# angelowxx/Super_resolution-Image-Reconstructer-Multi_Generator_GAN

Hardware: NVIDIA B200
Metric: srgan_train_lr_patches_per_sec (higher is better)
Workload: dtype bf16

## Files before the change

super_resolution-image-reconstructer-multi_generator_gan_b200/_lib.py:

```python
from __future__ import annotations

import ctypes
import os
import subprocess
from ctypes import POINTER, c_char_p, c_double, c_float, c_int, c_int64, c_longlong, c_size_t, c_void_p

HERE = os.path.dirname(os.path.abspath(__file__))
ROOT = os.path.dirname(HERE)
CSRC = os.path.join(HERE, "csrc")
SO_PATH = os.environ.get("SRG_LIB_SO") or os.path.join(HERE, "libsrgan_b200.so")
SOURCES = ["conv_gemm.cu", "conv_ops.cu", "vgg_ops.cu", "resample.cu", "trunk_fused.cu", "wgrad_gemm.cu", "elementwise.cu", "peer_sync.cu", "generator.cu", "discriminator.cu", "api.cu"]
NVCC_FLAGS = ["-gencode", "arch=compute_100a,code=sm_100a", "-O3", "-lineinfo", "-std=c++17", "-shared",
              "-Xcompiler", "-fPIC"]

_lib = None


def _sources():
    return [os.path.join(CSRC, s) for s in SOURCES if os.path.exists(os.path.join(CSRC, s))]


def needs_build() -> bool:
    if os.environ.get("SRG_LIB_SO"):
        return False
    if not os.path.exists(SO_PATH):
        return True
    so_m = os.path.getmtime(SO_PATH)
    deps = _sources() + [os.path.join(CSRC, f) for f in os.listdir(CSRC) if f.endswith(".cuh")]
    deps.append(os.path.join(ROOT, "include", "srgan_b200.h"))
    return any(os.path.getmtime(d) > so_m for d in deps if os.path.exists(d))


def build(force: bool = False, verbose: bool = False) -> str:
    if not force and not needs_build():
        return SO_PATH
    nvcc = os.environ.get("NVCC", "/usr/local/cuda/bin/nvcc")
    cmd = [nvcc] + NVCC_FLAGS + ["-o", SO_PATH] + _sources() + ["-ldl"]
    if verbose:
        print(" ".join(cmd))
    r = subprocess.run(cmd, capture_output=True, text=True)
    if r.returncode != 0:
        raise RuntimeError("nvcc failed:\n" + r.stdout + r.stderr)
    return SO_PATH

# ... 146 lines not shown
```

super_resolution-image-reconstructer-multi_generator_gan_b200/csrc/conv_gemm.cu:

```cuda
#include "conv_gemm.cuh"
#include "elementwise.cuh"
#include "launch.cuh"
#include "ptx.cuh"

#include <stdarg.h>
#include <stdlib.h>
#include <stdio.h>
#include <string.h>

namespace srg {

static thread_local char g_err[512] = "";
const char* last_error() { return g_err; }
void set_error(const char* fmt, ...) {
  va_list ap;
  va_start(ap, fmt);
  vsnprintf(g_err, sizeof(g_err), fmt, ap);
  va_end(ap);
}

static long long g_launch_total = 0;
void count_launch(int n) { __atomic_fetch_add(&g_launch_total, (long long)n, __ATOMIC_RELAXED); }
long long total_launches() { return __atomic_load_n(&g_launch_total, __ATOMIC_RELAXED); }

// ... 1140 lines not shown
                                         227 * 1024);
    if (e != cudaSuccess) { set_error("cudaFuncSetAttribute: %s", cudaGetErrorString(e)); return int(e); }
    attr_set = true;
  }
  cudaError_t e = launch_pdl(conv_gemm_kernel<BLOCK_N, NT>, grid, dim3(kThreads), smem_bytes, stream, p);
  if (e == cudaSuccess) e = cudaGetLastError();
  if (e != cudaSuccess) { set_error("conv_gemm launch: %s", cudaGetErrorString(e)); return int(e); }
  count_launch();
  return 0;
}

static bool conv3_il_enabled() {
  static int on = -1;
  if (on < 0) {
    const char* ev = getenv("SRG_CONV_IL");
    on = (ev != nullptr && ev[0] == '0') ? 0 : 1;
  }
  return on != 0;
}
static bool conv3_il_wide_enabled() {
  static int on = -1;
  if (on < 0) {
    const char* ev = getenv("SRG_CONV_IL_WIDE");
    on = (ev != nullptr && ev[0] == '0') ? 0 : 1;
  }
  return on != 0;
}
static int g_variant_override = 0;
int set_conv_variant(int variant) {
  const int old = g_variant_override;
  g_variant_override = (variant >= 0 && variant <= 3) ? variant : 0;
  return old;
}
static int effective_variant(const ConvGemmArgs& a) { return a.variant != 0 ? a.variant : g_variant_override; }
static bool use_conv3_il(const ConvGemmArgs& a) {
  const int variant = effective_variant(a);
  if (variant == 1 || (variant == 0 && !conv3_il_enabled())) return false;
  return a.TH == 16 && a.TW == 8 && a.block_n == 64 && a.n_strips == 3 && a.n_taps == 3 && a.strip_dh == -1 &&
         a.strip_rows == 18 && a.tap_row[0] == 0 && a.tap_row[1] == 1 && a.tap_row[2] == 2 && a.n_views == 1 &&
         a.views[0].channels == 64 && a.in_H == a.H && a.in_W == a.W && a.H >= 2 &&
         (a.out_mode == OUT_NHWC || a.out_mode == OUT_PIXEL_SHUFFLE) &&
         a.cout_total % 64 == 0 && a.cout_total <= 256;
}

static int encode_parity_map(CUtensorMap* map, const void* base, int C, int W, int H, int N, int64_t stride_w,
                             int64_t stride_h, int64_t stride_n, int par, uint32_t box_rows, uint32_t box_w = 8) {
  const __nv_bfloat16* ptr = reinterpret_cast<const __nv_bfloat16*>(base) + size_t(par) * stride_h;
  uint64_t dims[4] = {uint64_t(C), uint64_t(W), uint64_t((H - par + 1) / 2), uint64_t(N)};
  uint64_t strides[3] = {uint64_t(stride_w) * 2, uint64_t(stride_h) * 4, uint64_t(stride_n) * 2};
  uint32_t box[4] = {64, box_w, box_rows, 1};
  return encode_map_bf16(map, ptr, 4, dims, strides, box);
}

static int launch_conv3_il(const ConvGemmArgs* as, int n, cudaStream_t stream) {
  const ConvGemmArgs& a = as[0];
  if (n < 1 || n > kIlMaxGroups) { set_error("conv3_il: 1..%d groups", kIlMaxGroups); return -17; }
  for (int g = 1; g < n; ++g) {
    const ConvGemmArgs& o = as[g];
    if (o.N != a.N || o.H != a.H || o.W != a.W || o.in_H != a.in_H || o.in_W != a.in_W || o.cout_total != 64 || a.cout_total != 64 ||
        o.out_mode != OUT_NHWC || a.out_mode != OUT_NHWC || o.act != a.act || o.slope != a.slope || o.exclusive != a.exclusive ||
        (o.residual != nullptr) != (a.residual != nullptr) || (o.mask_src != nullptr) != (a.mask_src != nullptr) ||
        (o.stats != nullptr) != (a.stats != nullptr) || (o.stats_y != nullptr) != (a.stats_y != nullptr) ||
        o.views[0].stride_w != a.views[0].stride_w || o.views[0].stride_h != a.views[0].stride_h ||
        o.views[0].stride_n != a.views[0].stride_n || o.strip_dw[0] != a.strip_dw[0] || o.strip_dw[1] != a.strip_dw[1] ||
        o.strip_dw[2] != a.strip_dw[2] || effective_variant(o) != effective_variant(a) || a.prof != nullptr) {
      set_error("conv3_il: the problems of a grouped launch must share geometry, epilogue and layout (OUT_NHWC, 64 channels)");
// ... 349 lines not shown
```

super_resolution-image-reconstructer-multi_generator_gan_b200/csrc/conv_gemm.cuh:

```cuda
#pragma once
#include <cuda.h>
#include <cuda_bf16.h>
#include <cuda_runtime.h>
#include <stdint.h>

namespace srg {

constexpr int kMaxStrips = 9;
constexpr int kMaxTaps = 9;
constexpr int kMaxInMaps = 4;

enum ConvAct : int { ACT_NONE = 0, ACT_RELU = 1, ACT_LRELU = 2 };
enum ConvOutMode : int {
  OUT_NHWC = 0,
  OUT_PIXEL_SHUFFLE = 1,
  OUT_FOLD9_NCHW = 2,
  OUT_NHWC_F32 = 3,
};

struct InView {
  const void* ptr;
  int64_t stride_w;
  int64_t stride_h;
  int64_t stride_n;
// ... 50 lines not shown
};
int wgrad_partials_floats(const WgradArgs& a, int* splits_out);
int launch_wgrad_gemm(const WgradArgs& a, cudaStream_t stream);
int wgrad3x3_partials_floats(const WgradArgs& a, int* splits_out);
int launch_wgrad3x3(const WgradArgs& a, cudaStream_t stream);
struct WgradBatchArgs {
  int N, H, W, n_layers;
  const void* x_base;
  int64_t x_layer_stride_bytes;
  const void* dy_base;
  int64_t dy_layer_stride_bytes;
  float* partials;
  const int* inv;
  float* grads;
  const long long* out_off;
};
void wgrad3_batched_plan(const WgradBatchArgs& a, int* tiles_per_layer, int* grid, int* per_cta, int* max_slots);
size_t wgrad3_batched_partials_floats(const WgradBatchArgs& a);
int launch_wgrad3x3_batched(const WgradBatchArgs& a, cudaStream_t stream);
int launch_wgrad_reduce(const float* partials, const int* idx, float* out, int n_out, int splits, size_t split_stride,
                        int accumulate_into, cudaStream_t stream);

struct C9Window { int jlo, jhi, slot_lo, fresh; };
__host__ __device__ inline C9Window c9_window(int ri) {
  C9Window w;
  w.jlo = ri > 8 ? ri - 8 : 0;
  w.jhi = ri < 7 ? ri : 7;
  w.slot_lo = 8 - ri + w.jlo;
  w.fresh = ri <= 7 ? 1 : 0;
  return w;
}

int set_conv_variant(int variant);

int sm_budget();
void set_sm_share(int k);

void count_launch(int n = 1);
long long total_launches();

int launch_wgrad_reduce_inv(const float* partials, const int* inv, float* out, int n_part, int splits, size_t split_stride,
                            cudaStream_t stream);

const char* last_error();
void set_error(const char* fmt, ...);

}
```

super_resolution-image-reconstructer-multi_generator_gan_b200/csrc/generator.cu:

```cuda
#include "generator.cuh"

#include <stdio.h>
#include <stdlib.h>
#include <string.h>

#include "conv_gemm.cuh"
#include "elementwise.cuh"
#include "peer_sync.cuh"
#include "trunk_fused.cuh"

namespace srg {

namespace {

constexpr float kBnEps = 1e-5f;
constexpr float kBnMomentum = 0.1f;
constexpr float kSlope = 0.2f;

struct Carver {
  size_t off = 0;
  size_t take(size_t bytes) {
    const size_t o = off;
    off += (bytes + 1023) & ~size_t(1023);
    return o;
  }
};

struct Layout {
  size_t packed, bias, bncoef, bwdcoef, partials, sums, ticket, wg_partials, ps_scratch, loss_scratch;
  size_t dyall = 0, slot = 0;
  size_t wgb_partials = 0, wgb_floats = 0;
  size_t trunk_sync = 0, trunk_tab = 0;
  size_t U1, out1, trunk;
  std::vector<size_t> y1, z1, y2, out;
  std::vector<size_t> up;
  size_t g[4];
  std::vector<size_t> dup;
  size_t Ud;
// ... 40 lines not shown
    }
  } else {
    const size_t y1 = c.take(t64(P)), z1 = c.take(t64(P)), y2 = c.take(t64(P)), oa = c.take(t64(P)), ob = c.take(t64(P));
    for (int b = 0; b < e.n_res; ++b) { L.y1[b] = y1; L.z1[b] = z1; L.y2[b] = y2; L.out[b] = (b & 1) ? ob : oa; }
  }
  L.trunk = c.take(t64(P));
  L.up.resize(e.n_up);
  for (int j = 0; j < e.n_up; ++j) L.up[j] = c.take(t64(P << (2 * (j + 1))));
  L.wg_partials = L.ps_scratch = L.loss_scratch = L.Ud = 0;
  for (int i = 0; i < 4; ++i) L.g[i] = 0;
  L.dup.assign(e.n_up, 0);
  if (training) {
    L.wg_partials = c.take(size_t(wgrad_max_floats(e.n_up)) * 4);
    L.ps_scratch = c.take(size_t(e.N) * (size_t(e.H) << e.n_up) * 128 * 4);
    L.loss_scratch = c.take(size_t(loss_scratch_doubles()) * 8);
    for (int i = 0; i < 3; ++i) L.g[i] = c.take(t64(P));
    L.slot = (t64(P) + 1023) & ~size_t(1023);
    L.dyall = c.take(L.slot * size_t(2 * e.n_res + 1));
    L.g[3] = L.dyall + L.slot * size_t(2 * e.n_res);
    L.kd_last = L.kd_c1 = 0;
    if (e.keep_grads) {
      L.kd_y2.resize(e.n_res); L.kd_p1.resize(e.n_res); L.kd_y1.resize(e.n_res); L.kd_in.resize(e.n_res);
      for (int b = 0; b < e.n_res; ++b) {
        L.kd_y2[b] = L.dyall + L.slot * size_t(2 * b + 1); L.kd_y1[b] = L.dyall + L.slot * size_t(2 * b);
        L.kd_p1[b] = c.take(t64(P)); L.kd_in[b] = c.take(t64(P));
      }
      L.kd_last = c.take(t64(P));
      L.kd_c1 = c.take(t64(P));
    }
    L.wgb_floats = wgrad_batched_floats(e);
    L.wgb_partials = c.take(L.wgb_floats * 4);
    for (int j = 0; j < e.n_up; ++j) L.dup[j] = c.take(t64(P << (2 * (j + 1))));
    const int64_t Hs = int64_t(e.H) << e.n_up, Ws = int64_t(e.W) << e.n_up;
    L.Ud = c.take(size_t(e.N) * (Hs + 1) * Ws * 128);
  }
  L.total = c.off;
  return L;
}

int64_t add_param(GeneratorEngine& e, const std::string& name, std::initializer_list<int> shape) {
  ParamInfo p;
  p.name = name;
  p.ndim = int(shape.size());
  p.numel = 1;
  int i = 0;
  for (int s : shape) { p.shape[i++] = s; p.numel *= s; }
  for (; i < 4; ++i) p.shape[i] = 1;
  p.offset = e.param_elems;
  e.param_elems += (p.numel + 3) & ~int64_t(3);
  e.params.push_back(p);
  return p.offset;
}
int64_t poff(const GeneratorEngine& e, const std::string& name) {
  for (const auto& p : e.params)
    if (p.name == name) return p.offset;
  return -1;
}
int64_t boff(const GeneratorEngine& e, const std::string& name) {
  for (const auto& b : e.buffers)
    if (b.name == name) return b.offset;
  return -1;
}

struct PackOffsets {
  int64_t conv1_f;
  std::vector<int64_t> rb_f[2], rb_d[2];
  int64_t conv2_f, conv2_d;
// ... 579 lines not shown
  for (size_t i = 0; i + 1 < g->prof_used; i += 2) {
    cudaError_t e = cudaEventSynchronize(g->prof_events[i + 1]);
    if (e != cudaSuccess) { set_error("profile_read: %s", cudaGetErrorString(e)); return int(e); }
    float ms = 0.f;
    e = cudaEventElapsedTime(&ms, g->prof_events[i], g->prof_events[i + 1]);
    if (e != cudaSuccess) { set_error("profile_read: %s", cudaGetErrorString(e)); return int(e); }
    total += double(ms);
  }
  if (ms_sum) *ms_sum = total;
  if (count) *count = (long long)(g->prof_used / 2);
  g->prof_used = 0;
  return 0;
}

GeneratorEngine::~GeneratorEngine() {
  for (cudaEvent_t ev : prof_events) cudaEventDestroy(ev);
  cudaFree(d_pack_idx); cudaFree(d_bias_idx); cudaFree(d_wg_idx_c3x3); cudaFree(d_wg_idx_up);
  cudaFree(d_wg_idx_conv1); cudaFree(d_wg_idx_conv3); cudaFree(d_wgb_off);
}

GeneratorEngine* generator_create(int N, int H, int W, int n_res, int n_up) {
  if (N < 1 || H < 1 || W < 1 || n_res < 0 || n_up < 0 || n_up > 4) { set_error("generator_create: bad geometry"); return nullptr; }
  EngineImpl* e = new EngineImpl();
  e->N = N; e->H = H; e->W = W; e->n_res = n_res; e->n_up = n_up;
  {
    const char* ev = getenv("SRG_FUSE_BWD_STATS");
    e->fuse_bwd_stats = ev != nullptr && ev[0] == '1';
    ev = getenv("SRG_REDUCE_FINAL");
    e->reduce_final = ev != nullptr && ev[0] == '1';
    ev = getenv("SRG_FIN_FUSED");
    e->fin_fused = ev != nullptr && ev[0] == '1';
    ev = getenv("SRG_WGRAD_BATCHED");
    e->wgrad_batched = !(ev != nullptr && ev[0] == '0');
  }
  add_param(*e, "conv1.weight", {64, 3, 9, 9});
  add_param(*e, "conv1.bias", {64});
  char nm[96];
  for (int b = 0; b < n_res; ++b) {
    const char* sub[2][2] = {{"conv1", "bn1"}, {"conv2", "bn2"}};
    for (int k = 0; k < 2; ++k) {
      snprintf(nm, sizeof(nm), "residual_blocks.%d.%s.weight", b, sub[k][0]); add_param(*e, nm, {64, 64, 3, 3});
      snprintf(nm, sizeof(nm), "residual_blocks.%d.%s.bias", b, sub[k][0]); add_param(*e, nm, {64});
      snprintf(nm, sizeof(nm), "residual_blocks.%d.%s.weight", b, sub[k][1]); add_param(*e, nm, {64});
      snprintf(nm, sizeof(nm), "residual_blocks.%d.%s.bias", b, sub[k][1]); add_param(*e, nm, {64});
      for (const char* stat : {"running_mean", "running_var"}) {
        BufferInfo bi;
        snprintf(nm, sizeof(nm), "residual_blocks.%d.%s.%s", b, sub[k][1], stat);
        bi.name = nm; bi.offset = e->buffer_elems; bi.numel = 64;
        e->buffer_elems += 64;
        e->buffers.push_back(bi);
      }
    }
  }
  add_param(*e, "conv2.weight", {64, 64, 3, 3});
  add_param(*e, "conv2.bias", {64});
  for (int j = 0; j < n_up; ++j) {
    snprintf(nm, sizeof(nm), "upsample.%d.weight", 3 * j); add_param(*e, nm, {256, 64, 3, 3});
    snprintf(nm, sizeof(nm), "upsample.%d.bias", 3 * j); add_param(*e, nm, {256});
  }
  add_param(*e, "conv3.weight", {3, 64, 9, 9});
  add_param(*e, "conv3.bias", {3});

  std::vector<int> idx;
  idx.reserve(size_t(e->param_elems) * 2 + 65536);
  PackOffsets& po = e->po;
  po.conv1_f = int64_t(idx.size()); pack_conv1_fwd(idx, poff(*e, "conv1.weight"));
// ... 405 lines not shown
    return launch_wgrad_reduce_inv(wgp, idx, e->grads + pi->offset, int(per_split), splits, per_split, st);
  };
  auto bias_grad = [&](const void* dy, int64_t pixels, const std::string& bname) -> int {
    ReduceFinalize f; memset(&f, 0, sizeof(f));
    f.mode = RF_SUM; f.count = double(pixels); f.out0 = e->grads + poff(*e, bname);
    RC(launch_chan_reduce(dy, nullptr, pixels, partials, st));
    e->launches += 2;
    return launch_partials_finalize(partials, reduce_blocks(pixels), f, st);
  };
  int bwd_stats_rows = 0;
  auto dgrad3x3 = [&](const void* dy_base, int gh, int gw, bool dy_ps, int64_t w_off, const void* residual, const void* mask,
                      void* out, const void* stats_y) -> int {
    ConvGemmArgs a; memset(&a, 0, sizeof(a));
    a.N = N; a.H = gh; a.W = gw; set_taps_3x3(a);
    if (dy_ps) {
      a.n_views = 4;
      for (int q = 0; q < 4; ++q) a.views[q] = ps_view(dy_base, gh, gw, q);
    } else {
      a.n_views = 1; a.views[0] = plain_view(dy_base, gh, gw);
    }
    a.in_H = gh; a.in_W = gw;
    a.weights = packed + w_off; a.cout_total = 64; a.block_n = 64;
    a.bias = nullptr; a.act = ACT_NONE; a.residual = residual; a.mask_src = mask; a.out = out; a.out_mode = OUT_NHWC;
    if (stats_y != nullptr && e->fuse_bwd_stats) { a.stats = partials; a.stats_y = stats_y; bwd_stats_rows = conv_gemm_grid(a); }
    e->launches += 1;
    if (dy_ps) return launch_conv_gemm(a, st);
    ProfScope ps(e, st);
    return launch_conv_gemm(a, st);
  };

  const void* conv3_in = S > 0 ? ws + L.up[S - 1] : ws + L.trunk;
  void* d_trunk = ws + L.g[3];
  if (pre) {
  RC(launch_unfold9(dsr, N, Hs, Ws, 1.f, ws + L.Ud, st));
  RC(launch_nchw_chan_sum(dsr, N, 3, int64_t(Hs) * Ws, reinterpret_cast<double*>(ws + L.loss_scratch),
                          e->grads + poff(*e, "conv3.bias"), 1.f, st));
  e->launches += 3;
  {
    InView uv = plain_view(ws + L.Ud, Hs + 1, Ws);
    RC(wgrad(uv, Hs + 1, Ws, true, Hs, Ws, conv3_in, 1, false, e->d_wg_idx_conv3, "conv3.weight"));
  }
  {
    ConvGemmArgs a; memset(&a, 0, sizeof(a));
    a.N = N; a.H = Hs; a.W = Ws; set_taps_pairs(a);
    a.n_views = 1; a.views[0] = plain_view(ws + L.Ud, Hs + 1, Ws); a.in_H = Hs + 1; a.in_W = Ws;
    a.weights = packed + po.conv3_d; a.cout_total = 64; a.block_n = 64;
    a.act = ACT_NONE; a.out_mode = OUT_NHWC;
    a.mask_src = S > 0 ? conv3_in : nullptr;
    a.out = S > 0 ? ws + L.dup[S - 1] : d_trunk;
    RC(launch_conv_gemm(a, st));
    e->launches += 1;
  }
  for (int j = S - 1; j >= 0; --j) {
    const int Hj = H << j, Wj = W << j;
    const void* in_j = j > 0 ? ws + L.up[j - 1] : ws + L.trunk;
    snprintf(nm, sizeof(nm), "upsample.%d.bias", 3 * j);
    RC(launch_ps_bias_grad(ws + L.dup[j], N, Hj * 2, Wj * 2, reinterpret_cast<float*>(ws + L.ps_scratch),
                           e->grads + poff(*e, nm), st));
    e->launches += 2;
    snprintf(nm, sizeof(nm), "upsample.%d.weight", 3 * j);
    RC(wgrad(plain_view(in_j, Hj, Wj), Hj, Wj, false, Hj, Wj, ws + L.dup[j], 4, true, e->d_wg_idx_up, nm));
    RC(dgrad3x3(ws + L.dup[j], Hj, Wj, true, po.up_d[j], nullptr, j > 0 ? in_j : nullptr, j > 0 ? ws + L.dup[j - 1] : d_trunk, nullptr));
  }
  }
  const void* x_last = e->n_res > 0 ? ws + L.out[e->n_res - 1] : ws + L.out1;
  if (pre) RC(bias_grad(d_trunk, P, "conv2.bias"));
  bool batched = e->wgrad_batched && e->n_res > 0;
  for (int b = 0; b < e->n_res && batched; ++b) {
    const size_t x1 = b > 0 ? L.out[b - 1] : L.out1;
    if (x1 != L.out1 + size_t(2 * b) * 2 * L.slot || L.z1[b] != L.out1 + size_t(2 * b + 1) * 2 * L.slot) batched = false;
  }
  if (batched && L.out[e->n_res - 1] != L.out1 + size_t(2 * e->n_res) * 2 * L.slot) batched = false;
  if (batched) {
    WgradBatchArgs probe; memset(&probe, 0, sizeof(probe));
    probe.N = N; probe.H = H; probe.W = W; probe.n_layers = 2 * e->n_res + 1;
    if (wgrad3_batched_partials_floats(probe) > L.wgb_floats) batched = false;
  }
  if (!batched && pre) RC(wgrad(plain_view(x_last, H, W), H, W, false, H, W, d_trunk, 1, false, e->d_wg_idx_c3x3, "conv2.weight"));
  const bool keep = e->keep_grads;
  void* dout = keep ? ws + L.kd_last : ws + L.g[0];
  void* dother = ws + L.g[1];
  void* dmid = ws + L.g[2];
  const bool fused = batched && use_trunk_fused(*e);
  const bool layers_here = !fused && phases == kPhaseAll;
// ... 91 lines not shown
```

super_resolution-image-reconstructer-multi_generator_gan_b200/csrc/generator.cuh:

```cuda
#pragma once
#include <cuda_runtime.h>
#include <stdint.h>

#include <string>
#include <vector>

namespace srg {

struct ParamInfo {
  std::string name;
  int64_t offset;
  int64_t numel;
  int ndim;
  int shape[4];
};
struct BufferInfo {
  std::string name;
  int64_t offset;
  int64_t numel;
};
struct TensorInfo {
  std::string name;
  int64_t byte_offset;
  int dims[4];
// ... 2 lines not shown

typedef int (*AllreduceF64Fn)(void* ctx, double* buf, int n, cudaStream_t stream);

struct GeneratorEngine {
  int N, H, W, n_res, n_up;
  std::vector<ParamInfo> params;
  std::vector<BufferInfo> buffers;
  std::vector<TensorInfo> tensors;
  int64_t param_elems = 0, buffer_elems = 0;
  int64_t packed_elems = 0, bias_elems = 0;
  size_t workspace_bytes_train = 0, workspace_bytes_eval = 0;
  int* d_pack_idx = nullptr;
  int* d_bias_idx = nullptr;
  int* d_wg_idx_c3x3 = nullptr;
  int* d_wg_idx_up = nullptr;
  int* d_wg_idx_conv1 = nullptr;
  int* d_wg_idx_conv3 = nullptr;
  long long* d_wgb_off = nullptr;
  float* master = nullptr;
  float* grads = nullptr;
  float* bn_buffers = nullptr;
  uint8_t* ws = nullptr;
  size_t ws_bytes = 0;
  bool ws_training = false;
  AllreduceF64Fn allreduce = nullptr;
  void* allreduce_ctx = nullptr;
  struct PeerSync* peer = nullptr;
  int world = 1;
  long long launches = 0;
  bool fuse_bwd_stats = false;
  bool fin_fused = false;
  bool reduce_final = false;
  bool wgrad_batched = true;
  bool keep_grads = false;
  bool prof_on = false;
  std::vector<cudaEvent_t> prof_events;
  size_t prof_used = 0;
  int prof_layers = 1;

  virtual ~GeneratorEngine();
};

GeneratorEngine* generator_create(int N, int H, int W, int n_res, int n_up);
int generator_bind(GeneratorEngine* g, float* master, float* grads, float* bn_buffers, void* ws, size_t ws_bytes,
                   int training);
int generator_pack(GeneratorEngine* g, cudaStream_t st);
int generator_forward(GeneratorEngine* g, const float* lr_nchw, float* sr_nchw, int training, int update_running,
                      cudaStream_t st);
int generator_backward(GeneratorEngine* g, const float* dsr_nchw, cudaStream_t st);
enum GeneratorPhase : int { kPhasePre = 1, kPhaseTrunk = 2, kPhasePost = 4, kPhaseAll = 7 };
int generator_forward_phases(GeneratorEngine* g, const float* lr_nchw, float* sr_nchw, int training, int update_running,
                             int phases, cudaStream_t st);
int generator_backward_phases(GeneratorEngine* g, const float* dsr_nchw, int phases, cudaStream_t st);
int generators_trunk(GeneratorEngine* const* gs, int n, int bwd, int update_running, cudaStream_t st);
int generator_set_keep_grads(GeneratorEngine* g, int keep);
int generator_trunk_error(GeneratorEngine* g);
int generator_prof_layers(const GeneratorEngine* g);
int generator_profile_enable(GeneratorEngine* g, int on);
int generator_profile_read(GeneratorEngine* g, double* ms_sum, long long* count);

}
```

Before: 1702.

## Fuse conv3 backward unfold into dedicated dgrad and wgrad tcgen05 kernels

New measurement: 1750, median of 6. +2.8%, better.

```diff
diff --git a/super_resolution-image-reconstructer-multi_generator_gan_b200/_lib.py b/super_resolution-image-reconstructer-multi_generator_gan_b200/_lib.py
--- a/super_resolution-image-reconstructer-multi_generator_gan_b200/_lib.py
+++ b/super_resolution-image-reconstructer-multi_generator_gan_b200/_lib.py
@@ -9,7 +9,7 @@
 ROOT = os.path.dirname(HERE)
 CSRC = os.path.join(HERE, "csrc")
 SO_PATH = os.environ.get("SRG_LIB_SO") or os.path.join(HERE, "libsrgan_b200.so")
-SOURCES = ["conv_gemm.cu", "conv_ops.cu", "vgg_ops.cu", "resample.cu", "trunk_fused.cu", "wgrad_gemm.cu", "elementwise.cu", "peer_sync.cu", "generator.cu", "discriminator.cu", "api.cu"]
+SOURCES = ["conv_gemm.cu", "conv_ops.cu", "vgg_ops.cu", "resample.cu", "trunk_fused.cu", "wgrad_gemm.cu", "conv9_bwd.cu", "elementwise.cu", "peer_sync.cu", "generator.cu", "discriminator.cu", "api.cu"]
 NVCC_FLAGS = ["-gencode", "arch=compute_100a,code=sm_100a", "-O3", "-lineinfo", "-std=c++17", "-shared",
               "-Xcompiler", "-fPIC"]
 
diff --git a/super_resolution-image-reconstructer-multi_generator_gan_b200/csrc/conv9_bwd.cu b/super_resolution-image-reconstructer-multi_generator_gan_b200/csrc/conv9_bwd.cu
--- /dev/null
+++ b/super_resolution-image-reconstructer-multi_generator_gan_b200/csrc/conv9_bwd.cu
@@ -0,0 +1,551 @@
+#include "conv9_bwd.cuh"
+#include "elementwise.cuh"
+#include "launch.cuh"
+#include "ptx.cuh"
+
+#include <string.h>
+
+namespace srg {
+
+int encode_map_bf16(CUtensorMap* map, const void* ptr, int rank, const uint64_t* dims, const uint64_t* strides_bytes,
+                    const uint32_t* box);
+
+namespace {
+
+constexpr int kTH = 16, kTW = 8;
+constexpr int kStripRows = 24;
+constexpr uint32_t kStripBytes = kStripRows * kTW * 128;
+constexpr uint32_t kTileBytes = kTH * kTW * 128;
+constexpr int kWinRows = kStripRows + 1;
+constexpr int kWinCols = 16;
+constexpr int kWinPitch = 24;
+constexpr int kWinPlane = kWinRows * kWinPitch;
+constexpr int kWinLoads = 3 * kWinRows * kWinCols;
+constexpr uint32_t kWinBytes = 3 * kWinPlane * 4;
+constexpr int kBuilders = 192;
+constexpr int kPf = (kWinLoads + kBuilders - 1) / kBuilders;
+constexpr int kTaps = 5;
+constexpr uint32_t kWBytes = kTaps * 64 * 128;
+
+struct TileXY { int n, h0, w0; };
+__device__ __forceinline__ TileXY tile_xy(int tile, int tiles_w, int tiles_per_img) {
+  TileXY t;
+  t.n = tile / tiles_per_img;
+  const int rem = tile - t.n * tiles_per_img;
+  t.h0 = (rem / tiles_w) * kTH;
+  t.w0 = (rem % tiles_w) * kTW;
+  return t;
+}
+
+__device__ __forceinline__ void win_prefetch(float (&pf)[kPf], const float* __restrict__ dsr, int H, int W, int btid, TileXY t,
+                                             bool valid) {
+#pragma unroll
+  for (int k = 0; k < kPf; ++k) {
+    const int i = btid + k * kBuilders;
+    const int c = i / (kWinRows * kWinCols);
+    const int rem = i - c * (kWinRows * kWinCols);
+    const int r = rem / kWinCols, col = rem - r * kWinCols;
+    const int hh = t.h0 - 4 + r, ww = t.w0 - 4 + col;
+    pf[k] = (valid && i < kWinLoads && hh >= 0 && hh < H && ww >= 0 && ww < W)
+                ? __ldg(dsr + ((size_t(t.n) * 3 + c) * H + hh) * size_t(W) + ww) : 0.f;
+  }
+}
+__device__ __forceinline__ void win_store(const float (&pf)[kPf], float* win, int btid) {
+#pragma unroll
+  for (int k = 0; k < kPf; ++k) {
+    const int i = btid + k * kBuilders;
+    if (i < kWinLoads) {
+      const int c = i / (kWinRows * kWinCols);
+      const int rem = i - c * (kWinRows * kWinCols);
+      const int r = rem / kWinCols, col = rem - r * kWinCols;
+      win[c * kWinPlane + r * kWinPitch + col] = pf[k];
+    }
+  }
+}
+__device__ __forceinline__ void build_slot(const float* win, uint8_t* strip, int btid, bool col_ok) {
+  const int r = btid >> 3, x = btid & 7;
+  float f[64];
+#pragma unroll
+  for (int ch = 54; ch < 64; ++ch) f[ch] = 0.f;
+#pragma unroll
+  for (int dr = 0; dr < 2; ++dr)
+#pragma unroll
+    for (int c = 0; c < 3; ++c) {
+      const float* row = win + c * kWinPlane + (r + dr) * kWinPitch + x;
+#pragma unroll
+      for (int sft = 0; sft < 9; ++sft) f[dr * 27 + sft * 3 + c] = col_ok ? row[sft] : 0.f;
+    }
+  uint8_t* dst = strip + btid * 128;
+#pragma unroll
+  for (int g = 0; g < 8; ++g) {
+    uint4 v;
+    v.x = pack_bf16(f[8 * g + 0], f[8 * g + 1]); v.y = pack_bf16(f[8 * g + 2], f[8 * g + 3]);
+    v.z = pack_bf16(f[8 * g + 4], f[8 * g + 5]); v.w = pack_bf16(f[8 * g + 6], f[8 * g + 7]);
+    *reinterpret_cast<uint4*>(dst + ((g ^ x) << 4)) = v;
+  }
+}
+
+struct C9bKParams {
+  CUtensorMap x_map;
+  CUtensorMap w_map;
+  CUtensorMap out_map;
+  const float* dsr;
+  int N, H, W;
+  int tiles_w, tiles_per_img, tiles_total;
+  int n_ctas, n_stages;
+  int mask;
+  float* partials;
+  double* bias_partials;
+  uint64_t pol_in;
+};
+
+constexpr int kBarNamed = 5;
+
+template <bool BIAS>
+__device__ __forceinline__ void builder_loop(const C9bKParams& p, float* win, uint8_t* stages, uint32_t stage_bytes,
+                                             uint32_t strip_off, uint64_t* full, uint64_t* empty, int btid, int off0, int off1,
+                                             double& bs0, double& bs1) {
+  float pa[kPf], pb[kPf];
+  const int step2 = 2 * p.n_ctas;
+  int tile = blockIdx.x;
+  win_prefetch(pa, p.dsr, p.H, p.W, btid, tile_xy(tile, p.tiles_w, p.tiles_per_img), tile < p.tiles_total);
+  win_prefetch(pb, p.dsr, p.H, p.W, btid, tile_xy(tile + p.n_ctas, p.tiles_w, p.tiles_per_img), tile + p.n_ctas < p.tiles_total);
+  int stage = 0;
+  uint32_t phase = 0;
+  auto step = [&](float (&pf)[kPf], int tl) {
+    const TileXY t = tile_xy(tl, p.tiles_w, p.tiles_per_img);
+    named_bar_sync(kBarNamed, kBuilders);
+    win_store(pf, win, btid);
+    named_bar_sync(kBarNamed, kBuilders);
+    const int nxt = tl + step2;
+    win_prefetch(pf, p.dsr, p.H, p.W, btid, tile_xy(nxt, p.tiles_w, p.tiles_per_img), nxt < p.tiles_total);
+    if (BIAS) {
+      bs0 += double(win[off0]);
+      bs1 += double(win[off1]);
+    }
+    mbar_wait(&empty[stage], phase ^ 1);
+    build_slot(win, stages + size_t(stage) * stage_bytes + strip_off, btid, t.w0 + (btid & 7) < p.W);
+    fence_proxy_async_smem();
+    mbar_arrive(&full[stage]);
+    if (++stage == p.n_stages) { stage = 0; phase ^= 1; }
+  };
+  for (; tile < p.tiles_total; tile += step2) {
+    step(pa, tile);
+    if (tile + p.n_ctas < p.tiles_total) step(pb, tile + p.n_ctas);
+  }
+}
+
+constexpr int kDgThreads = 512;
+constexpr int kDgBuild0 = 320;
+
+__global__ void __launch_bounds__(kDgThreads, 1) conv9_bwd_dgrad_kernel(const __grid_constant__ C9bKParams p) {
+  extern __shared__ uint8_t smem_raw[];
+  uint8_t* smem = reinterpret_cast<uint8_t*>((reinterpret_cast<uintptr_t>(smem_raw) + 1023) & ~uintptr_t(1023));
+  __builtin_assume(__isShared(smem));
+  const int warp = uniform_warp_idx();
+  const int lane = threadIdx.x & 31;
+  pdl_trigger();
+
+  uint8_t* w_smem = smem;
+  uint8_t* stages = w_smem + kWBytes;
+  uint8_t* out_stage = stages + size_t(p.n_stages) * kStripBytes;
+  uint8_t* aux_stage = out_stage + 2 * kTileBytes;
+  float* win = reinterpret_cast<float*>(aux_stage + 2 * kTileBytes);
+  uint64_t* bars = reinterpret_cast<uint64_t*>(reinterpret_cast<uint8_t*>(win) + ((kWinBytes + 127) & ~127u));
+  uint64_t* full = bars;
+  uint64_t* empty = bars + 8;
+  uint64_t* wfull = bars + 16;
+  uint64_t* tfull = bars + 17;
+  uint64_t* tempty = bars + 19;
+  uint64_t* auxfull = bars + 21;
+  uint64_t* auxempty = bars + 23;
+  uint32_t* tmem_slot = reinterpret_cast<uint32_t*>(bars + 25);
+
+  if (warp == 0 && lane == 0) {
+    for (int i = 0; i < p.n_stages; ++i) {
+      mbar_init(&full[i], kBuilders);
+      mbar_init(&empty[i], 1);
+    }
+    mbar_init(wfull, 1);
+    for (int i = 0; i < 2; ++i) {
+      mbar_init(&tfull[i], 1);
+      mbar_init(&tempty[i], 256);
+      mbar_init(&auxfull[i], 1);
+      mbar_init(&auxempty[i], 256);
+    }
+    fence_barrier_init();
+    tma_prefetch_desc(&p.x_map);
+    tma_prefetch_desc(&p.w_map);
+    tma_prefetch_desc(&p.out_map);
+  }
+  if (warp == 1) tmem_alloc(tmem_slot, 128);
+  tc_fence_before();
+  __syncthreads();
+  tc_fence_after();
+  const uint32_t tmem_base = *tmem_slot;
+
+  if (warp == 0) {
+    if (elect_one()) {
+      mbar_expect_tx(wfull, kWBytes);
+      for (int kb = 0; kb < kTaps; ++kb) tma_load_2d(w_smem + size_t(kb) * 8192, &p.w_map, wfull, 0, kb * 64);
+      if (p.mask) {
+        pdl_wait();
+        int ab = 0;
+        uint32_t aux_phase = 0;
+        for (int tile = blockIdx.x; tile < p.tiles_total; tile += p.n_ctas) {
+          const TileXY t = tile_xy(tile, p.tiles_w, p.tiles_per_img);
+          mbar_wait(&auxempty[ab], aux_phase ^ 1);
+          mbar_expect_tx(&auxfull[ab], kTileBytes);
+          tma_load_4d_hint(aux_stage + ab * kTileBytes, &p.x_map, &auxfull[ab], 0, t.w0, t.h0, t.n, p.pol_in);
+          ab ^= 1;
+          if (ab == 0) aux_phase ^= 1;
+        }
+      }
+    }
+  } else if (warp == 1) {
+    constexpr uint32_t idesc = make_idesc_bf16(128, 64, 0, 0);
+    const uint64_t desc_hi = (uint64_t(1024 >> 4) << 32) | (uint64_t(1) << 46) | (uint64_t(2) << 61);
+    const uint32_t stage0_lo = smem_u32(stages) >> 4;
+    const uint32_t w_lo = smem_u32(w_smem) >> 4;
+    mbar_wait(wfull, 0);
+    int stage = 0, acc = 0;
+    uint32_t phase = 0, acc_phase = 0;
+    for (int tile = blockIdx.x; tile < p.tiles_total; tile += p.n_ctas) {
+      mbar_wait(&tempty[acc], acc_phase ^ 1);
+      tc_fence_after();
+      const uint32_t d_tmem = tmem_base + uint32_t(acc * 64);
+      mbar_wait(&full[stage], phase);
+      tc_fence_after();
+      const uint32_t a_lo = stage0_lo + uint32_t(stage) * (kStripBytes >> 4);
+      if (elect_one()) {
+        uint32_t accumulate = 0;
+#pragma unroll
+        for (int r = 0; r < kTaps; ++r) {
+          const uint64_t adesc = desc_hi | uint64_t(a_lo + uint32_t(2 * r * kTW) * 8u);
+          const uint64_t bdesc = desc_hi | uint64_t(w_lo + uint32_t(r) * (8192 >> 4));
+#pragma unroll
+          for (int k = 0; k < 4; ++k) {
+            umma_bf16(d_tmem, adesc + uint64_t(2 * k), bdesc + uint64_t(2 * k), idesc, accumulate);
+            accumulate = 1;
+          }
+        }
+        umma_commit(&empty[stage]);
+        umma_commit(&tfull[acc]);
+      }
+      __syncwarp();
+      if (++stage == p.n_stages) { stage = 0; phase ^= 1; }
+      acc ^= 1;
+      if (acc == 0) acc_phase ^= 1;
+    }
+  } else if (warp < 10) {
+    const int q = warp & 3;
+    const int m = q * 32 + lane;
+    const int hf = (warp - 2) >> 2;
+    const int etid = threadIdx.x - 64;
+    int acc = 0, ob = 0, ab = 0;
+    uint32_t acc_phase = 0, aux_phase = 0;
+    for (int tile = blockIdx.x; tile < p.tiles_total; tile += p.n_ctas) {
+      const TileXY t = tile_xy(tile, p.tiles_w, p.tiles_per_img);
+      mbar_wait(&tfull[acc], acc_phase);
+      tc_fence_after();
+      uint32_t v[32];
+      tmem_ld32(tmem_base + (uint32_t(q * 32) << 16) + uint32_t(acc * 64 + hf * 32), v);
+      tmem_ld_wait();
+      tc_fence_before();
+      mbar_arrive(&tempty[acc]);
+      float f[32];
+#pragma unroll
+      for (int j = 0; j < 32; ++j) f[j] = fmaf(__uint_as_float(v[j]), 1.f, 0.f);
+      const uint32_t row_off = uint32_t(m) * 128u;
+      const uint32_t sw = uint32_t(m & 7);
+      if (p.mask) {
+        mbar_wait(&auxfull[ab], aux_phase);
+        const uint8_t* ap = aux_stage + ab * kTileBytes + row_off;
+#pragma unroll
+        for (int g = 0; g < 4; ++g) {
+          const uint4 r = *reinterpret_cast<const uint4*>(ap + (((uint32_t(hf * 4 + g)) ^ sw) << 4));
+          const uint32_t ws[4] = {r.x, r.y, r.z, r.w};
+#pragma unroll
+          for (int e = 0; e < 4; ++e) {
+            if (!(bf16_lo(ws[e]) > 0.f)) f[g * 8 + 2 * e] = 0.f;
+            if (!(bf16_hi(ws[e]) > 0.f)) f[g * 8 + 2 * e + 1] = 0.f;
+          }
+        }
+        mbar_arrive(&auxempty[ab]);
+        ab ^= 1;
+        if (ab == 0) aux_phase ^= 1;
+      }
+      if (etid == 0) tma_store_wait_read<1>();
+      named_bar_sync(1, 256);
+      uint8_t* op = out_stage + ob * kTileBytes + row_off;
+#pragma unroll
+      for (int g = 0; g < 4; ++g) {
+        uint4 o;
+        o.x = pack_bf16(f[g * 8 + 0], f[g * 8 + 1]);
+        o.y = pack_bf16(f[g * 8 + 2], f[g * 8 + 3]);
+        o.z = pack_bf16(f[g * 8 + 4], f[g * 8 + 5]);
+        o.w = pack_bf16(f[g * 8 + 6], f[g * 8 + 7]);
+        *reinterpret_cast<uint4*>(op + (((uint32_t(hf * 4 + g)) ^ sw) << 4)) = o;
+      }
+      fence_proxy_async_smem();
+      named_bar_sync(2, 256);
+      if (etid == 0) {
+        tma_store_4d(&p.out_map, out_stage + ob * kTileBytes, 0, t.w0, t.h0, t.n);
+        tma_store_commit();
+      }
+      ob ^= 1;
+      acc ^= 1;
+      if (acc == 0) acc_phase ^= 1;
+    }
+    if (etid == 0) tma_store_wait_all<0>();
+  } else {
+    const int btid = threadIdx.x - kDgBuild0;
+    pdl_wait();
+    double unused0 = 0.0, unused1 = 0.0;
+    builder_loop<false>(p, win, stages, kStripBytes, 0, full, empty, btid, 0, 0, unused0, unused1);
+  }
+  tc_fence_before();
+  __syncthreads();
+  if (warp == 1) tmem_dealloc(tmem_base, 128);
+}
+
+constexpr int kWgThreads9 = 384;
+constexpr int kWgBuild0 = 192;
+constexpr int kXRows = kTH + 4;
+constexpr uint32_t kXStripBytes = kXRows * kTW * 128;
+constexpr uint32_t kWgStage = kXStripBytes + kStripBytes;
+
+__global__ void __launch_bounds__(kWgThreads9, 1) conv9_bwd_wgrad_kernel(const __grid_constant__ C9bKParams p) {
+  extern __shared__ uint8_t smem_raw[];
+  uint8_t* smem = reinterpret_cast<uint8_t*>((reinterpret_cast<uintptr_t>(smem_raw) + 1023) & ~uintptr_t(1023));
+  __builtin_assume(__isShared(smem));
+  const int warp = uniform_warp_idx();
+  const int lane = threadIdx.x & 31;
+  pdl_trigger();
+
+  uint8_t* stages = smem;
+  float* win = reinterpret_cast<float*>(stages + size_t(p.n_stages) * kWgStage);
+  uint64_t* bars = reinterpret_cast<uint64_t*>(reinterpret_cast<uint8_t*>(win) + ((kWinBytes + 127) & ~127u));
+  uint64_t* full = bars;
+  uint64_t* empty = bars + 8;
+  uint64_t* done = bars + 16;
+  uint32_t* tmem_slot = reinterpret_cast<uint32_t*>(bars + 17);
+
+  if (warp == 0 && elect_one()) {
+    for (int i = 0; i < p.n_stages; ++i) {
+      mbar_init(&full[i], kBuilders + 1);
+      mbar_init(&empty[i], 1);
+    }
+    mbar_init(done, 1);
+    fence_barrier_init();
+    tma_prefetch_desc(&p.x_map);
+  }
+  if (warp == 1) tmem_alloc(tmem_slot, 256);
+  tc_fence_before();
+  __syncthreads();
+  tc_fence_after();
+  const uint32_t tmem_base = *tmem_slot;
+
+  if (warp == 0) {
+    if (elect_one()) {
+      pdl_wait();
+      int stage = 0;
+      uint32_t phase = 0;
+      for (int tile = blockIdx.x; tile < p.tiles_total; tile += p.n_ctas) {
+        const TileXY t = tile_xy(tile, p.tiles_w, p.tiles_per_img);
+        mbar_wait(&empty[stage], phase ^ 1);
+        mbar_expect_tx(&full[stage], kXStripBytes);
+        tma_load_4d_hint(stages + size_t(stage) * kWgStage, &p.x_map, &full[stage], 0, t.w0, t.h0 - 4, t.n, p.pol_in);
+        if (++stage == p.n_stages) { stage = 0; phase ^= 1; }
+      }
+    }
+  } else if (warp == 1) {
+    constexpr uint32_t idesc = make_idesc_bf16(128, 192, 1, 1);
+    const uint64_t hi_common = (uint64_t(1024 >> 4) << 32) | (uint64_t(1) << 46) | (uint64_t(2) << 61);
+    const uint64_t a_hi = hi_common | (uint64_t(((6 * kTW * 128) >> 4) & 0x3FFF) << 16);
+    const uint64_t b_hi = hi_common | (uint64_t(((2 * kTW * 128) >> 4) & 0x3FFF) << 16);
+    int stage = 0;
+    uint32_t phase = 0;
+    uint32_t accumulate = 0;
+    for (int tile = blockIdx.x; tile < p.tiles_total; tile += p.n_ctas) {
+      mbar_wait(&full[stage], phase);
+      tc_fence_after();
+      const uint32_t base = smem_u32(stages + size_t(stage) * kWgStage);
+      if (elect_one()) {
+        const uint64_t bdesc = b_hi | uint64_t(base >> 4);
+        const uint64_t adesc = a_hi | uint64_t((base + kXStripBytes) >> 4);
+#pragma unroll
+        for (int k = 0; k < 8; ++k)
+          umma_bf16(tmem_base, adesc + uint64_t(128 * k), bdesc + uint64_t(128 * k), idesc, (k > 0) ? 1u : accumulate);
+        umma_commit(&empty[stage]);
+      }
+      __syncwarp();
+      accumulate = 1;
+      if (++stage == p.n_stages) { stage = 0; phase ^= 1; }
+    }
+    if (elect_one()) umma_commit(done);
+    __syncwarp();
+  } else if (warp < 6) {
+    const int q = warp & 3;
+    const int m = q * 32 + lane;
+    pdl_wait();
+    mbar_wait(done, 0);
+    tc_fence_after();
+    const bool any = int(blockIdx.x) < p.tiles_total;
+    float* dst = p.partials + size_t(blockIdx.x) * 3 * 128 * 64;
+    const bool lo = q < 2;
+    const int k = m & 63;
+    for (int i = 0; i < 3; ++i) {
+      const int t = lo ? 2 - i : 5 - i;
+      const bool keep = any && t < 5;
+      float* row = dst + (size_t(t < 5 ? t >> 1 : 2) * 128 + (t < 5 ? (t & 1) * 64 : 64) + k) * 64;
+#pragma unroll
+      for (int half = 0; half < 2; ++half) {
+        uint32_t v[32];
+        tmem_ld32(tmem_base + (uint32_t(q * 32) << 16) + uint32_t(i * 64 + half * 32), v);
+        tmem_ld_wait();
+        float4* o = reinterpret_cast<float4*>(row + half * 32);
+#pragma unroll
+        for (int g = 0; g < 8; ++g) {
+          float4 f;
+          f.x = keep ? __uint_as_float(v[4 * g + 0]) : 0.f;
+          f.y = keep ? __uint_as_float(v[4 * g + 1]) : 0.f;
+          f.z = keep ? __uint_as_float(v[4 * g + 2]) : 0.f;
+          f.w = keep ? __uint_as_float(v[4 * g + 3]) : 0.f;
+          o[g] = f;
+        }
+      }
+    }
+  } else {
+    const int btid = threadIdx.x - kWgBuild0;
+    const int j0 = btid, j1 = btid + kBuilders;
+    const int off0 = (j0 >> 7) * kWinPlane + (4 + ((j0 & 127) >> 3)) * kWinPitch + 4 + (j0 & 7);
+    const int off1 = (j1 >> 7) * kWinPlane + (4 + ((j1 & 127) >> 3)) * kWinPitch + 4 + (j1 & 7);
+    double bs0 = 0.0, bs1 = 0.0;
+    pdl_wait();
+    builder_loop<true>(p, win, stages, kWgStage, kXStripBytes, full, empty, btid, off0, off1, bs0, bs1);
+    double* red = reinterpret_cast<double*>(win);
+    named_bar_sync(kBarNamed, kBuilders);
+    red[j0] = bs0;
+    red[j1] = bs1;
+    named_bar_sync(kBarNamed, kBuilders);
+    if (btid < 3) {
+      double s = 0.0;
+      for (int j = 0; j < 128; ++j) s += red[btid * 128 + j];
+      p.bias_partials[size_t(blockIdx.x) * 3 + btid] = s;
+    }
+  }
+  tc_fence_before();
+  __syncthreads();
+  if (warp == 1) tmem_dealloc(tmem_base, 256);
+}
+
+__global__ void c9_bias_final_kernel(const double* __restrict__ partials, int rows, float* __restrict__ dbias) {
+  pdl_trigger();
+  pdl_wait();
+  const int c = threadIdx.x;
+  if (c >= 3) return;
+  double s = 0.0;
+  for (int r = 0; r < rows; ++r) s += partials[size_t(r) * 3 + c];
+  dbias[c] = float(s);
+}
+
+int tile_rows(int H, bool wgrad) { return (H + (wgrad ? 4 : 0) + kTH - 1) / kTH; }
+
+int fill_common(C9bKParams& p, const Conv9BwdArgs& a, bool wgrad) {
+  memset(&p, 0, sizeof(p));
+  p.N = a.N; p.H = a.H; p.W = a.W;
+  p.tiles_w = (a.W + kTW - 1) / kTW;
+  p.tiles_per_img = p.tiles_w * tile_rows(a.H, wgrad);
+  p.tiles_total = a.N * p.tiles_per_img;
+  p.dsr = a.dsr;
+  p.n_ctas = sm_budget() < p.tiles_total ? sm_budget() : p.tiles_total;
+  if (p.n_ctas < 1) p.n_ctas = 1;
+  uint64_t dims[4] = {64, uint64_t(a.W), uint64_t(a.H), uint64_t(a.N)};
+  uint64_t strides[3] = {128, uint64_t(a.W) * 128, uint64_t(a.H) * a.W * 128};
+  uint32_t box[4] = {64, uint32_t(kTW), uint32_t(wgrad ? kXRows : kTH), 1};
+  return encode_map_bf16(&p.x_map, a.x, 4, dims, strides, box);
+}
+
+}
+
+int conv9_bwd_ctas(int N, int H, int W) {
+  const int tiles = N * tile_rows(H, true) * ((W + kTW - 1) / kTW);
+  const int s = sm_budget() < tiles ? sm_budget() : tiles;
+  return s < 1 ? 1 : s;
+}
+
+int launch_conv9_bwd_dgrad(const Conv9BwdArgs& a, cudaStream_t stream) {
+  C9bKParams p;
+  {
+    const int rc = fill_common(p, a, false);
+    if (rc) return rc;
+  }
+  if (p.tiles_total == 0) return 0;
+  p.mask = a.mask ? 1 : 0;
+  p.pol_in = l2_hints() >= 2 ? kL2EvictFirst : kL2EvictNormal;
+  {
+    uint64_t dims[2] = {64, uint64_t(kTaps) * 64};
+    uint64_t strides[1] = {128};
+    uint32_t box[2] = {64, 64};
+    const int rc = encode_map_bf16(&p.w_map, a.w_dgrad, 2, dims, strides, box);
+    if (rc) return rc;
+  }
+  {
+    uint64_t dims[4] = {64, uint64_t(a.W), uint64_t(a.H), uint64_t(a.N)};
+    uint64_t strides[3] = {128, uint64_t(a.W) * 128, uint64_t(a.H) * a.W * 128};
+    uint32_t box[4] = {64, uint32_t(kTW), uint32_t(kTH), 1};
+    const int rc = encode_map_bf16(&p.out_map, a.dx, 4, dims, strides, box);
+    if (rc) return rc;
+  }
+  const uint32_t fixed = kWBytes + 4 * kTileBytes + ((kWinBytes + 127) & ~127u) + 256;
+  int stages = int((227u * 1024u - 1024u - fixed) / kStripBytes);
+  if (stages > 8) stages = 8;
+  p.n_stages = stages;
+  const size_t smem_bytes = 1024 + fixed + size_t(stages) * kStripBytes;
+  static DeviceOnce attr;
+  if (!attr) {
+    cudaError_t e = cudaFuncSetAttribute(conv9_bwd_dgrad_kernel, cudaFuncAttributeMaxDynamicSharedMemorySize, 227 * 1024);
+    if (e != cudaSuccess) { set_error("cudaFuncSetAttribute: %s", cudaGetErrorString(e)); return int(e); }
+    attr = true;
+  }
+  cudaError_t e = launch_pdl(conv9_bwd_dgrad_kernel, dim3(p.n_ctas), dim3(kDgThreads), smem_bytes, stream, p);
+  if (e == cudaSuccess) e = cudaGetLastError();
+  if (e != cudaSuccess) { set_error("conv9_bwd_dgrad launch: %s", cudaGetErrorString(e)); return int(e); }
+  count_launch();
+  return 0;
+}
+
+int launch_conv9_bwd_wgrad(const Conv9BwdArgs& a, cudaStream_t stream) {
+  C9bKParams p;
+  {
+    const int rc = fill_common(p, a, true);
+    if (rc) return rc;
+  }
+  if (p.tiles_total == 0) return 0;
+  p.partials = a.partials;
+  p.bias_partials = a.bias_partials;
+  p.pol_in = l2_hints() >= 4 ? kL2EvictFirst : kL2EvictNormal;
+  const uint32_t fixed = ((kWinBytes + 127) & ~127u) + 256;
+  int stages = int((227u * 1024u - 1024u - fixed) / kWgStage);
+  if (stages > 4) stages = 4;
+  p.n_stages = stages;
+  const size_t smem_bytes = 1024 + fixed + size_t(stages) * kWgStage;
+  static DeviceOnce attr;
+  if (!attr) {
+    cudaError_t e = cudaFuncSetAttribute(conv9_bwd_wgrad_kernel, cudaFuncAttributeMaxDynamicSharedMemorySize, 227 * 1024);
+    if (e != cudaSuccess) { set_error("cudaFuncSetAttribute: %s", cudaGetErrorString(e)); return int(e); }
+    attr = true;
+  }
+  cudaError_t e = launch_pdl(conv9_bwd_wgrad_kernel, dim3(p.n_ctas), dim3(kWgThreads9), smem_bytes, stream, p);
+  if (e == cudaSuccess) e = cudaGetLastError();
+  if (e != cudaSuccess) { set_error("conv9_bwd_wgrad launch: %s", cudaGetErrorString(e)); return int(e); }
+  count_launch();
+  e = launch_pdl(c9_bias_final_kernel, dim3(1), dim3(32), 0, stream, static_cast<const double*>(a.bias_partials), p.n_ctas, a.dbias);
+  if (e == cudaSuccess) e = cudaGetLastError();
+  if (e != cudaSuccess) { set_error("c9_bias_final launch: %s", cudaGetErrorString(e)); return int(e); }
+  count_launch();
+  return 0;
+}
+
+}
diff --git a/super_resolution-image-reconstructer-multi_generator_gan_b200/csrc/conv9_bwd.cuh b/super_resolution-image-reconstructer-multi_generator_gan_b200/csrc/conv9_bwd.cuh
--- /dev/null
+++ b/super_resolution-image-reconstructer-multi_generator_gan_b200/csrc/conv9_bwd.cuh
@@ -0,0 +1,22 @@
+#pragma once
+#include "conv_gemm.cuh"
+
+namespace srg {
+
+struct Conv9BwdArgs {
+  int N, H, W;
+  const float* dsr;
+  const void* x;
+  int mask;
+  const void* w_dgrad;
+  void* dx;
+  float* partials;
+  double* bias_partials;
+  float* dbias;
+};
+
+int conv9_bwd_ctas(int N, int H, int W);
+int launch_conv9_bwd_dgrad(const Conv9BwdArgs& a, cudaStream_t stream);
+int launch_conv9_bwd_wgrad(const Conv9BwdArgs& a, cudaStream_t stream);
+
+}
diff --git a/super_resolution-image-reconstructer-multi_generator_gan_b200/csrc/conv_gemm.cu b/super_resolution-image-reconstructer-multi_generator_gan_b200/csrc/conv_gemm.cu
--- a/super_resolution-image-reconstructer-multi_generator_gan_b200/csrc/conv_gemm.cu
+++ b/super_resolution-image-reconstructer-multi_generator_gan_b200/csrc/conv_gemm.cu
@@ -1196,6 +1196,7 @@
   g_variant_override = (variant >= 0 && variant <= 3) ? variant : 0;
   return old;
 }
+int conv_variant() { return g_variant_override; }
 static int effective_variant(const ConvGemmArgs& a) { return a.variant != 0 ? a.variant : g_variant_override; }
 static bool use_conv3_il(const ConvGemmArgs& a) {
   const int variant = effective_variant(a);
diff --git a/super_resolution-image-reconstructer-multi_generator_gan_b200/csrc/conv_gemm.cuh b/super_resolution-image-reconstructer-multi_generator_gan_b200/csrc/conv_gemm.cuh
--- a/super_resolution-image-reconstructer-multi_generator_gan_b200/csrc/conv_gemm.cuh
+++ b/super_resolution-image-reconstructer-multi_generator_gan_b200/csrc/conv_gemm.cuh
@@ -106,6 +106,7 @@
 }
 
 int set_conv_variant(int variant);
+int conv_variant();
 
 int sm_budget();
 void set_sm_share(int k);
diff --git a/super_resolution-image-reconstructer-multi_generator_gan_b200/csrc/generator.cu b/super_resolution-image-reconstructer-multi_generator_gan_b200/csrc/generator.cu
--- a/super_resolution-image-reconstructer-multi_generator_gan_b200/csrc/generator.cu
+++ b/super_resolution-image-reconstructer-multi_generator_gan_b200/csrc/generator.cu
@@ -4,6 +4,7 @@
 #include <stdlib.h>
 #include <string.h>
 
+#include "conv9_bwd.cuh"
 #include "conv_gemm.cuh"
 #include "elementwise.cuh"
 #include "peer_sync.cuh"
@@ -110,7 +111,7 @@
     L.wgb_partials = c.take(L.wgb_floats * 4);
     for (int j = 0; j < e.n_up; ++j) L.dup[j] = c.take(t64(P << (2 * (j + 1))));
     const int64_t Hs = int64_t(e.H) << e.n_up, Ws = int64_t(e.W) << e.n_up;
-    L.Ud = c.take(size_t(e.N) * (Hs + 1) * Ws * 128);
+    if (!e.c9_bwd) L.Ud = c.take(size_t(e.N) * (Hs + 1) * Ws * 128);
   }
   L.total = c.off;
   return L;
@@ -756,6 +757,8 @@
     e->fin_fused = ev != nullptr && ev[0] == '1';
     ev = getenv("SRG_WGRAD_BATCHED");
     e->wgrad_batched = !(ev != nullptr && ev[0] == '0');
+    ev = getenv("SRG_C9_BWD");
+    e->c9_bwd = !(ev != nullptr && ev[0] == '0') && conv_variant() != 1;
   }
   add_param(*e, "conv1.weight", {64, 3, 9, 9});
   add_param(*e, "conv1.bias", {64});
@@ -1227,24 +1230,44 @@
   const void* conv3_in = S > 0 ? ws + L.up[S - 1] : ws + L.trunk;
   void* d_trunk = ws + L.g[3];
   if (pre) {
-  RC(launch_unfold9(dsr, N, Hs, Ws, 1.f, ws + L.Ud, st));
-  RC(launch_nchw_chan_sum(dsr, N, 3, int64_t(Hs) * Ws, reinterpret_cast<double*>(ws + L.loss_scratch),
-                          e->grads + poff(*e, "conv3.bias"), 1.f, st));
-  e->launches += 3;
-  {
-    InView uv = plain_view(ws + L.Ud, Hs + 1, Ws);
-    RC(wgrad(uv, Hs + 1, Ws, true, Hs, Ws, conv3_in, 1, false, e->d_wg_idx_conv3, "conv3.weight"));
-  }
-  {
-    ConvGemmArgs a; memset(&a, 0, sizeof(a));
-    a.N = N; a.H = Hs; a.W = Ws; set_taps_pairs(a);
-    a.n_views = 1; a.views[0] = plain_view(ws + L.Ud, Hs + 1, Ws); a.in_H = Hs + 1; a.in_W = Ws;
-    a.weights = packed + po.conv3_d; a.cout_total = 64; a.block_n = 64;
-    a.act = ACT_NONE; a.out_mode = OUT_NHWC;
-    a.mask_src = S > 0 ? conv3_in : nullptr;
-    a.out = S > 0 ? ws + L.dup[S - 1] : d_trunk;
-    RC(launch_conv_gemm(a, st));
-    e->launches += 1;
+  if (e->c9_bwd) {
+    Conv9BwdArgs c; memset(&c, 0, sizeof(c));
+    c.N = N; c.H = Hs; c.W = Ws; c.dsr = dsr; c.x = conv3_in;
+    c.mask = S > 0 ? 1 : 0;
+    c.w_dgrad = packed + po.conv3_d;
+    c.dx = S > 0 ? ws + L.dup[S - 1] : d_trunk;
+    c.partials = wgp;
+    c.bias_partials = reinterpret_cast<double*>(ws + L.loss_scratch);
+    c.dbias = e->grads + poff(*e, "conv3.bias");
+    const int splits = conv9_bwd_ctas(N, Hs, Ws);
+    const size_t per_split = size_t(3) * 128 * 64;
+    if (int64_t(splits) * int64_t(per_split) > wgrad_max_floats(S) || splits * 3 > loss_scratch_doubles()) {
+      set_error("conv9_bwd: partials exceed workspace"); return -27;
+    }
+    RC(launch_conv9_bwd_wgrad(c, st));
+    RC(launch_wgrad_reduce_inv(wgp, e->d_wg_idx_conv3, e->grads + poff(*e, "conv3.weight"), int(per_split), splits, per_split, st));
+    RC(launch_conv9_bwd_dgrad(c, st));
+    e->launches += 4;
+  } else {
+    RC(launch_unfold9(dsr, N, Hs, Ws, 1.f, ws + L.Ud, st));
+    RC(launch_nchw_chan_sum(dsr, N, 3, int64_t(Hs) * Ws, reinterpret_cast<double*>(ws + L.loss_scratch),
+                            e->grads + poff(*e, "conv3.bias"), 1.f, st));
+    e->launches += 3;
+    {
+      InView uv = plain_view(ws + L.Ud, Hs + 1, Ws);
+      RC(wgrad(uv, Hs + 1, Ws, true, Hs, Ws, conv3_in, 1, false, e->d_wg_idx_conv3, "conv3.weight"));
+    }
+    {
+      ConvGemmArgs a; memset(&a, 0, sizeof(a));
+      a.N = N; a.H = Hs; a.W = Ws; set_taps_pairs(a);
+      a.n_views = 1; a.views[0] = plain_view(ws + L.Ud, Hs + 1, Ws); a.in_H = Hs + 1; a.in_W = Ws;
+      a.weights = packed + po.conv3_d; a.cout_total = 64; a.block_n = 64;
+      a.act = ACT_NONE; a.out_mode = OUT_NHWC;
+      a.mask_src = S > 0 ? conv3_in : nullptr;
+      a.out = S > 0 ? ws + L.dup[S - 1] : d_trunk;
+      RC(launch_conv_gemm(a, st));
+      e->launches += 1;
+    }
   }
   for (int j = S - 1; j >= 0; --j) {
     const int Hj = H << j, Wj = W << j;
diff --git a/super_resolution-image-reconstructer-multi_generator_gan_b200/csrc/generator.cuh b/super_resolution-image-reconstructer-multi_generator_gan_b200/csrc/generator.cuh
--- a/super_resolution-image-reconstructer-multi_generator_gan_b200/csrc/generator.cuh
+++ b/super_resolution-image-reconstructer-multi_generator_gan_b200/csrc/generator.cuh
@@ -58,6 +58,7 @@
   bool fin_fused = false;
   bool reduce_final = false;
   bool wgrad_batched = true;
+  bool c9_bwd = true;
   bool keep_grads = false;
   bool prof_on = false;
   std::vector<cudaEvent_t> prof_events;
```
